# NVIDIA-AI-IOT/redtail

Hardware: AMD Instinct MI355X
Metric: stereo pairs/sec, ResNet18-2D 1257x369 (higher is better)
Workload: dtype f32

## Files before the change

### redtail_amd/csrc/kernels/conv_split.hip.h

```cpp
#pragma once
#include <type_traits>
#include "common.hip.h"
#include "conv_mfma.hip.h"

namespace rt {

constexpr float kSplitScale = 2048.f;
constexpr float kSplitInv = 1.f / 2048.f;

struct S3Split {
    f16x4 hi, lo;
};
__device__ static __forceinline__ S3Split s3_split(f32x4 v) {
    S3Split s;
#ifdef HIPEMU
#pragma unroll
    for (int j = 0; j < 4; j++) {
        const _Float16 h = (_Float16)v[j];
        s.hi[j] = h;
        s.lo[j] = (_Float16)((v[j] - (float)h) * kSplitScale);
    }
#else
    unsigned h[2], l[2];
#pragma unroll
// ... 182 lines not shown
                for (int e = 0; e < 4; e++)
                    o[e] = apply_act_fast(fmaf(acc_c[4 * q + e], kSplitInv, acc_m[4 * q + e]) + (bias4[q][e] + rr[q][e]), decltype(ACT)::value);
                if constexpr (YIL) {
                    const unsigned vo = (inb && 8 * q + 4 * kg < p.Cout) ? (unsigned)((oy * p.y_ystride + ox) * 4 + 4 * kg * cs32) * 4u : kBufOOB;
                    buf_store4(o, rs_y, vo, (unsigned)(8 * q * cs32) * 4u);
                } else {
                    const unsigned vo = inb ? (unsigned)(oy * p.y_ystride + ox * p.y_xstride + 4 * kg * cs32) * 4u : kBufOOB;
#pragma unroll
                    for (int e = 0; e < 4; e++)
                        buf_store(o[e], rs_y, (8 * q + 4 * kg + e < p.Cout) ? vo : kBufOOB, (unsigned)((8 * q + e) * cs32) * 4u);
                }
            }
        };
        if (act == 1) epilogue(std::integral_constant<int, 1>{});
        else if (act == 2) epilogue(std::integral_constant<int, 2>{});
        else epilogue(std::integral_constant<int, 0>{});
        RT_TSTAMP();
    }
#ifdef RT_KERNEL_TIMING
    __builtin_amdgcn_s_waitcnt(0);
    if (dbgp && tid == 0) { dbgp[14] = __builtin_amdgcn_s_memtime(); dbgp[15] = __builtin_amdgcn_s_memrealtime() - rt0; }
#endif
}

}

namespace rt {

template <int KH, int KW, int S, int NW_ = 4>
struct S3Cfg {
    static constexpr int NW = NW_, TY = NW_, TX = 32, CC = 16, TAPS = KH * KW, NT = 64 * NW_;
    static constexpr int PR = (TY - 1) * S + KH, PC = (TX - 1) * S + KW;
    static constexpr int PCH = (PC + 1) / 2;
    static constexpr int PCL = S == 2 ? 2 * PCH : PC;
    static constexpr int NPART = NW / 4;
    static constexpr int NPIX = PR * PC, NKP = ((NPIX + NPART - 1) / NPART + 63) / 64;
    static constexpr int PXB = 80;
    static constexpr int W_SLOTS = TAPS * 2 * 2 * 32;
    static constexpr int NK_W = (W_SLOTS + NT - 1) / NT;
    static constexpr int IN_BYTES = PR * PCL * PXB, GRP_BYTES = IN_BYTES + W_SLOTS * 16;
    static constexpr int KS_MAX = NW_ != 4 ? 1 : (S == 2 ? 2 : 4);
    static constexpr int max_groups(int want) {
        int ks = want < 1 ? 1 : (want > KS_MAX ? KS_MAX : want);
        while (ks > 1 && (ks == 3 || ks * GRP_BYTES < (ks - 1) * NW * 64 * 16 * 4)) ks--;
        return ks;
    }
    static_assert(IN_BYTES % 16 == 0, "weight image alignment");
    static_assert(S == 1 || S == 2, "stride 1 or 2");
};

#ifndef RT_S3_WAVES
#define RT_S3_WAVES(S) ((S) == 2 ? 2 : 4)
#endif
template <int KH, int KW, int S, bool XIL, bool YIL, int NW = 4, typename TIN = float, typename TOUT = float>
__global__ void __launch_bounds__(64 * NW * (S3Cfg<KH, KW, S, NW>::KS_MAX)) RT_WAVES_PER_EU(RT_S3_WAVES(S)) conv_s3_kernel(ConvArgs p) {
    using Cfg = S3Cfg<KH, KW, S, NW>;
    constexpr bool XF16 = std::is_same<TIN, _Float16>::value, YF16 = std::is_same<TOUT, _Float16>::value;
    constexpr unsigned ESX = Io<TIN>::ES, ESY = Io<TOUT>::ES;
    static_assert(!XIL || !XF16, "interleaved fp16 input: conv_f16mma_kernel");
    constexpr int TY = Cfg::TY, TX = Cfg::TX, CC = Cfg::CC, TAPS = Cfg::TAPS, PC = Cfg::PC, PCL = Cfg::PCL, PXB = Cfg::PXB;
    constexpr int NKP = Cfg::NKP, NK_W = Cfg::NK_W, NT = Cfg::NT;

    constexpr int IN_BYTES = Cfg::IN_BYTES, GRP_BYTES = Cfg::GRP_BYTES;
#ifdef HIPEMU
    HIP_DYNAMIC_SHARED(char, smem)
#else
    extern __shared__ __attribute__((aligned(16))) char smem[];
#endif

    const int tid_wg = threadIdx.x;
    const int KS = Cfg::KS_MAX == 1 ? 1 : __builtin_amdgcn_readfirstlane((int)blockDim.x / NT);
    const int kgi = Cfg::KS_MAX == 1 ? 0 : __builtin_amdgcn_readfirstlane(tid_wg / NT);
    const int tid = tid_wg - kgi * NT;
    char* const sIn = smem + kgi * GRP_BYTES;
    f32x4* const sW = reinterpret_cast<f32x4*>(smem + kgi * GRP_BYTES + IN_BYTES);
#ifdef RT_KERNEL_TIMING
    unsigned long long* dbgp = (p.dbg && kgi == 0) ? p.dbg + ((size_t)(blockIdx.z * gridDim.y + blockIdx.y) * gridDim.x + blockIdx.x) * 16 : nullptr;
    int dbi = 0;
    const unsigned long long rt0 = __builtin_amdgcn_s_memrealtime();
#endif
    RT_TSTAMP();
    const int lane = tid & 63;
    const int kg = lane >> 5, l31 = lane & 31;
    const int wv = __builtin_amdgcn_readfirstlane(tid >> 6);

    RT_WG_TILE_NB(p, tile, zi, n, nblk)
    const int tx0 = (tile % p.tiles_x) * TX;
    const int ty0 = (tile / p.tiles_x) * TY;
    const char* __restrict__ xb = elem_ptr(p.x, (int64_t)n * p.x_bstride, ESX);
    const int nchunks = p.CinPad / CC;
    int pad_y = p.pad_y, pad_x = p.pad_x, Ho = p.Ho, Wo = p.Wo, ch_row = zi;
    int64_t y_off = p.y_off + (int64_t)zi * p.y_zstride, w_off = 0, r_off = y_off, r_off_il8 = y_off;
    int64_t y_off_il4 = 4 * p.y_off + (int64_t)zi * p.y_zstride, r_off_il4 = y_off_il4;
    unsigned tap_mask = ~0u;
    if (p.zs) {
        const ZSlice z = p.zs[zi];
        pad_y = z.pad_y; pad_x = z.pad_x; Ho = z.Ho; Wo = z.Wo; ch_row = z.ch_row; y_off = z.y_off; w_off = z.w_off;
        r_off = z.r_off; r_off_il8 = z.r_off_il8;
        y_off_il4 = 4 * z.y_off;
        r_off_il4 = z.r_off_il4;
        tap_mask = z.tap_mask;
    }
    const int act = p.act;

    const int sg = wv & 3, spart = wv >> 2;
    const int* __restrict__ tab = p.ch_off + (int64_t)ch_row * p.CinPad + 4 * sg;
    unsigned voff[NKP];
    int lidx[NKP], xcol[NKP];
    const int* __restrict__ shtab = p.ch_shift ? p.ch_shift + (int64_t)ch_row * p.CinPad + 4 * sg : nullptr;
#pragma unroll
    for (int k = 0; k < NKP; k++) {
        const int pidx = spart * (NKP * 64) + lane + 64 * k;
        const int pr = pidx / PC, pc = pidx - pr * PC;
        const int iy = ty0 * S - pad_y + pr, ix = tx0 * S - pad_x + pc;
        const bool own = pidx < Cfg::NPIX && lane + 64 * k < NKP * 64;
        xcol[k] = ix;
        voff[k] = (own && iy >= 0 && iy < p.Hi && ix >= 0 && ix < p.Wi) ? (unsigned)(iy * p.x_pitch + ix) * (XIL ? 16u : ESX) : kBufOOB;
        const int col = S == 2 ? (pc & 1) * Cfg::PCH + (pc >> 1) : pc;
        lidx[k] = own ? (pr * PCL + col) * PXB + sg * 8 : -1;
    }
    const char* __restrict__ wsrc = reinterpret_cast<const char*>(p.w) + (w_off + ((int64_t)nblk * nchunks) * Cfg::W_SLOTS) * 16;
    const buf_rsrc rs_w = make_buf(wsrc);

    f32x4 rin[NKP];
    f32x4 rw[NK_W];
// ... 61 lines not shown
        const buf_rsrc rs_r = make_buf(elem_ptr(p.resid, r_il ? (int64_t)n * p.r_bstride + (YF16 ? r_off_il8 : r_off_il4) : rbase, ESY));
        if (r_il && YF16) {
            const unsigned vo = inb ? (unsigned)((oy * p.y_ystride + ox * p.y_xstride) * 8 + 4 * kg) * 2u : kBufOOB;
#pragma unroll
            for (int q = 0; q < 4; q++) {
                const u32x2_t u = __builtin_amdgcn_raw_buffer_load_b64(rs_r, (cb + 8 * q + 4 * kg < p.Cout) ? vo : kBufOOB, (unsigned)((cb + 8 * q) * rs32) * 2u, 0);
#pragma unroll
                for (int e = 0; e < 4; e++) rr[q][e] = (float)__builtin_bit_cast(_Float16, (unsigned short)(u[e >> 1] >> (16 * (e & 1))));
            }
        } else if (r_il) {
            const unsigned vo = inb ? (unsigned)((oy * p.y_ystride + ox * p.y_xstride) * 4 + 4 * kg * rs32) * 4u : kBufOOB;
#pragma unroll
            for (int q = 0; q < 4; q++) rr[q] = buf_load4(rs_r, (cb + 8 * q + 4 * kg < p.Cout) ? vo : kBufOOB, (unsigned)((cb + 8 * q) * rs32) * 4u);
        } else {
            const unsigned vo = inb ? (unsigned)(oy * p.y_ystride + ox * p.y_xstride + 4 * kg * rs32) * ESY : kBufOOB;
#pragma unroll
            for (int q = 0; q < 4; q++)
#pragma unroll
                for (int e = 0; e < 4; e++)
                    rr[q][e] = Io<TOUT>::load(rs_r, (cb + 8 * q + 4 * kg + e < p.Cout) ? vo : kBufOOB, (unsigned)((cb + 8 * q + e) * rs32) * ESY);
        }
    } else {
#pragma unroll
        for (int q = 0; q < 4; q++) rr[q] = f32x4{0.f, 0.f, 0.f, 0.f};
    }

    f32x16 acc_m, acc_c;
#pragma unroll
    for (int r = 0; r < 16; r++) { acc_m[r] = 0.f; acc_c[r] = 0.f; }
    const int a_off = kg * 32 + l31;
    const bool w_exact = p.w_exact != 0;
    const int b_off = (wv * S * PCL + l31) * PXB + kg * 16;
    auto compute = [&]() {
#pragma unroll
        for (int t = 0; t < TAPS; t++) {
            if (!((tap_mask >> t) & 1u)) continue;
            const int r = t / KW, s = t % KW;
            const int col = S == 2 ? (s & 1) * Cfg::PCH + (s >> 1) : s;
            const char* bp = sIn + b_off + (r * PCL + col) * PXB;
            const f16x8 bh = *reinterpret_cast<const f16x8*>(bp);
            const f16x8 ah = __builtin_bit_cast(f16x8, sW[a_off + (t * 2 + 0) * 64]);
            acc_m = __builtin_amdgcn_mfma_f32_32x32x16_f16(ah, bh, acc_m, 0, 0, 0);
            if (!w_exact) {
                const f16x8 al = __builtin_bit_cast(f16x8, sW[a_off + (t * 2 + 1) * 64]);
                acc_c = __builtin_amdgcn_mfma_f32_32x32x16_f16(al, bh, acc_c, 0, 0, 0);
            }
            if constexpr (!XF16) {
                const f16x8 bl = *reinterpret_cast<const f16x8*>(bp + 32);
                acc_c = __builtin_amdgcn_mfma_f32_32x32x16_f16(ah, bl, acc_c, 0, 0, 0);
            }
        }
    };

    if (kgi < nchunks) prefetch(kgi);
    RT_TSTAMP();
    for (int ch = kgi; ch < nchunks + kgi; ch += KS) {
        const bool mine = KS == 1 || ch < nchunks;
        if (ch != kgi) __syncthreads();
        if (mine) stage_to_lds();
        __syncthreads();
        RT_TSTAMP();
        if (ch + KS < nchunks) prefetch(ch + KS);
        if (mine) compute();
        RT_TSTAMP();
    }

#pragma unroll
    for (int r = 0; r < 16; r++) acc_m[r] = fmaf(acc_c[r], kSplitInv, acc_m[r]);
    if (KS > 1) {
        f32x4* const red = reinterpret_cast<f32x4*>(smem);
        __syncthreads();
        if (kgi > 0) {
#pragma unroll
            for (int q = 0; q < 4; q++)
                red[(((kgi - 1) * NW + wv) * 4 + q) * 64 + lane] = f32x4{acc_m[4 * q], acc_m[4 * q + 1], acc_m[4 * q + 2], acc_m[4 * q + 3]};
        }
        __syncthreads();
        if (kgi > 0) return;
        for (int g = 1; g < KS; g++)
#pragma unroll
            for (int q = 0; q < 4; q++) {
                const f32x4 v = red[(((g - 1) * NW + wv) * 4 + q) * 64 + lane];
#pragma unroll
                for (int e = 0; e < 4; e++) acc_m[4 * q + e] += v[e];
            }
    }

    const buf_rsrc rs_y = make_buf(elem_ptr(p.y, (YIL && !YF16) ? (int64_t)n * p.y_bstride + y_off_il4 : ybase, ESY));
    auto epilogue = [&](auto ACT) {
#pragma unroll
        for (int q = 0; q < 4; q++) {
            const f32x4 bv = *reinterpret_cast<const f32x4*>(p.bias + cb + 8 * q + 4 * kg);
            f32x4 o;
#pragma unroll
            for (int e = 0; e < 4; e++)
                o[e] = apply_act_fast(acc_m[4 * q + e] + (bv[e] + rr[q][e]), decltype(ACT)::value);
            if constexpr (YIL && YF16) {
                const unsigned vo = (inb && cb + 8 * q + 4 * kg < p.Cout) ? (unsigned)((oy * p.y_ystride + ox * p.y_xstride) * 8 + 4 * kg) * 2u : kBufOOB;
                u32x2_t w2;
#pragma unroll
                for (int e = 0; e < 2; e++)
                    w2[e] = (unsigned)__builtin_bit_cast(unsigned short, (_Float16)o[2 * e]) | ((unsigned)__builtin_bit_cast(unsigned short, (_Float16)o[2 * e + 1]) << 16);
                __builtin_amdgcn_raw_buffer_store_b64(w2, rs_y, vo, (unsigned)((cb + 8 * q) * cs32) * 2u, 0);
            } else if constexpr (YIL) {
                const unsigned vo = (inb && cb + 8 * q + 4 * kg < p.Cout) ? (unsigned)((oy * p.y_ystride + ox * p.y_xstride) * 4 + 4 * kg * cs32) * 4u : kBufOOB;
                buf_store4(o, rs_y, vo, (unsigned)((cb + 8 * q) * cs32) * 4u);
            } else {
                const unsigned vo = inb ? (unsigned)(oy * p.y_ystride + ox * p.y_xstride + 4 * kg * cs32) * ESY : kBufOOB;
#pragma unroll
                for (int e = 0; e < 4; e++)
                    Io<TOUT>::store(o[e], rs_y, (cb + 8 * q + 4 * kg + e < p.Cout) ? vo : kBufOOB, (unsigned)((cb + 8 * q + e) * cs32) * ESY);
            }
        }
    };
    if (act == 1) epilogue(std::integral_constant<int, 1>{});
    else if (act == 2) epilogue(std::integral_constant<int, 2>{});
    else epilogue(std::integral_constant<int, 0>{});
    RT_TSTAMP();
// ... 392 lines not shown
```

### redtail_amd/csrc/rt_capi.hip

```cpp
#include <hip/hip_runtime.h>

#include <algorithm>
#include <atomic>
#include <cmath>
#include <cstdarg>
#include <cstdio>
#include <cstdlib>
#include <cstring>
#include <string>
#include <map>
#include <mutex>
#include <vector>

#include "../../include/rt_stereo.h"
#if defined(__HIP_DEVICE_COMPILE__) && !defined(RT_BUILT_NO_SLP)
#error "rt_capi.hip must be compiled with -fno-slp-vectorize -DRT_BUILT_NO_SLP (redtail_amd/build.py: DEVICE_FLAGS)"
#endif
#include "kernels/common.hip.h"
#include "kernels/conv_mfma.hip.h"
#include "kernels/conv_wino.hip.h"
#include "kernels/deconv3d_small.hip.h"
#include "kernels/imgproc.hip.h"
#include "kernels/rectify.hip.h"
#include "kernels/decode.hip.h"
// ... 1063 lines not shown
namespace {


struct SubConv {
    int KH = 1, KW = 1, S = 1, NBW = 1, CC = 8;
    int TY = 4, TXW = 2, NW = 4, WLDS = 1;
    int CinPad = 0, Cout = 0;
    int Hi = 0, Wi = 0, Ho = 0, Wo = 0, pad_y = 0, pad_x = 0, nz = 1;
    int x_pitch = 0;
    std::vector<rt::ZSlice> zs_host;
    int64_t y_cstride = 0, y_zstride = 0, y_off = 0;
    int64_t r_cstride = 0;
    int y_ystride = 0, y_xstride = 1;
    float* w_dev = nullptr;
    int* choff_dev = nullptr;
    int w_exact = 0;
    int* shift_dev = nullptr;
    rt::ZSlice* zs_dev = nullptr;
    int direct = 0, cin_real = 0;
    int wino = 0;
    int x_f16 = 0, y_f16 = 0;
    int f16mma = 0;
    int x_il8 = 0, y_il8 = 0, r_il8 = 0;
    int dp4 = 0;
    int f16first = 0;
    int split3 = 0;
    int rb = 0;
    int s3first = 0;
    int s3p = 0;
    int small3d = 0;
    rt::Deconv3dSmallArgs s3{};
    std::vector<float> small_w;
    void* small_il_dev = nullptr;
    int small_il_f32 = 0;
};

}

struct FoldFactor {
    rtConvPlan* pl = nullptr;
    rtConvPlan* pr = nullptr;
    float* wedge_dev = nullptr;
    int F = 0, K = 0, D = 0, H = 0, W = 0;
    int64_t a_elems = 0, c_elems = 0, t_elems = 0, e_elems = 0;
    std::mutex mu;
    std::map<rtStream, std::pair<void*, size_t>> own;
};

struct ConvKnobs {
    int xcd = 1, trace = 0;
    int rb_tiles = 0;
    int rbs_seg = 0;
    int ksplit = -1;
    int s3p_grid = 0;
    int zinner = 1;
    int nbinner = 1;
    int dw = -1;
    int dw_nseg = 0;
    int fold_u = 2;
    int f16p_walk = -1;
    int f16p_classes = 1;
    int small_walk = -1;
    int r4 = -1;
};

struct rtConvPlan {
    std::vector<SubConv> subs;
    FoldFactor* ff = nullptr;
    mutable std::once_flag env_once;
    mutable ConvKnobs opt;
    int softarg = 0;
    float* bias_dev = nullptr;
    float* zeros_dev = nullptr;
    int act = 0, has_resid = 0, dtype = RT_F32;
    int out_dims[4] = {0, 0, 0, 1};
    int64_t x_bstride = 0, y_bstride = 0;
    int64_t r_bstride = 0;
    int is2d = 0, cin = 0, hin = 0, win = 0;
    std::vector<float> w_canon;
    rtConv2dDesc desc2d{};
    int is_deconv = 0;
    int in_pitch = 0, out_pitch = 0;
    float* rb_w1_dev = nullptr;
    float* rb_bias1_dev = nullptr;
    int rb_act1 = 0, rb_cmid = 0;
    float* rbd_w1_dev = nullptr;
    float* rbd_w2_dev = nullptr;
    int x_split = 0, y_split = 0;
    float* rbh_w1_dev = nullptr;
    float* rbh_w2_dev = nullptr;
    int w_f16 = 0;
    int is_conv3d = 0, is_deconv3d = 0;
    int c3d_C = 0, c3d_cin = 0, c3d_dchw = 0, c3d_fold = 0;
    int c3d_dw = 0;
    rtConv3dDesc desc3d{};
    int in_dims3[3] = {0, 0, 0};
    int flags = 0;
};

namespace {

struct Phase1D {
    int K = 0;
    int pad = 0;
    int tap[8] = {0};
};
// ... 117 lines not shown
                    const int nb = co / 32, cc = co % 32, ch = ci / 16, h = (ci % 16) / 8, e = ci % 8;
                    packed[(size_t)base * 8 + ((((((size_t)nb * nch + ch) * taps + (u * sc.KW + v)) * 2 + h) * 32 + cc) * 8) + e] = bits;
                }
    return base;
}

int upload_zslices(SubConv& sc, const std::vector<rt::ZSlice>& zs) {
    RT_HIP(hipMalloc((void**)&sc.zs_dev, zs.size() * sizeof(rt::ZSlice)));
    RT_HIP(hipMemcpy(sc.zs_dev, zs.data(), zs.size() * sizeof(rt::ZSlice), hipMemcpyHostToDevice));
    return 0;
}

int upload_table(SubConv& sc, const std::vector<int>& table) {
    RT_HIP(hipMalloc((void**)&sc.choff_dev, table.size() * sizeof(int)));
    RT_HIP(hipMemcpy(sc.choff_dev, table.data(), table.size() * sizeof(int), hipMemcpyHostToDevice));
    return 0;
}

int upload_bias(rtConvPlan* plan, const float* bias, int n) {
    const int padded = rt::round_up(n, 64);
    std::vector<float> b(padded + 64, 0.f);
    if (bias) std::memcpy(b.data(), bias, n * sizeof(float));
    RT_HIP(hipMalloc((void**)&plan->bias_dev, b.size() * sizeof(float)));
    RT_HIP(hipMemcpy(plan->bias_dev, b.data(), b.size() * sizeof(float), hipMemcpyHostToDevice));
    plan->zeros_dev = plan->bias_dev + padded;
    return 0;
}

bool window_supported(int KH, int KW, int S) {
    if (S == 1) return (KH == 3 && KW == 3) || (KH <= 2 && KW <= 2 && KH >= 1 && KW >= 1);
    if (S == 2) return (KH == 3 && KW == 3) || (KH == 5 && KW == 5);
    return false;
}

bool dev_knobs() {
    static const bool on = [] { const char* e = getenv("RT_DEV_KNOBS"); return e && atoi(e) != 0; }();
    return on;
}
int env_int(const char* name, int dflt) {
    if (!dev_knobs()) return dflt;
    const char* e = getenv(name);
    return e ? atoi(e) : dflt;
}

#ifdef RT_EXPERIMENTAL
inline int exp_knob(const char* name, int dflt) { return env_int(name, dflt); }
#else
inline int exp_knob(const char*, int dflt) { return dflt; }
#endif
ConvKnobs read_conv_knobs() {
    ConvKnobs k;
    k.xcd = env_int("RT_CONV_XCD", k.xcd); k.trace = env_int("RT_CONV_TRACE", k.trace);
    k.rb_tiles = exp_knob("RT_RB_TILES", k.rb_tiles); k.rbs_seg = env_int("RT_RBS_SEG", k.rbs_seg); k.ksplit = env_int("RT_S3_KSPLIT", k.ksplit);
    k.s3p_grid = env_int("RT_S3P_GRID", k.s3p_grid); k.zinner = env_int("RT_Z_INNER", k.zinner); k.nbinner = env_int("RT_NB_INNER", k.nbinner);
    k.dw = env_int("RT_F16_DW", k.dw); k.dw_nseg = env_int("RT_DW_NSEG", k.dw_nseg); k.fold_u = env_int("RT_FOLD_U", k.fold_u);
    k.f16p_walk = env_int("RT_F16P_WALK", k.f16p_walk); k.f16p_classes = env_int("RT_F16P_CLASSES", k.f16p_classes);
    k.small_walk = env_int("RT_SMALL_IL_WALK", k.small_walk); k.r4 = env_int("RT_F16_R4", k.r4);
    return k;
}
thread_local int tl_exact_fp32 = 0;
int exact_fp32() { return tl_exact_fp32 || env_int("RT_CONV_EXACT_FP32", 0) != 0; }
struct ExactScope {
    int prev;
    explicit ExactScope(int flags) : prev(tl_exact_fp32) { tl_exact_fp32 = (flags & RT_CONV_EXACT_FP32) ? 1 : prev; }
    ~ExactScope() { tl_exact_fp32 = prev; }
};

void set_tile(SubConv& sc, int variant) {
    switch (variant) {
        case 0: sc.TY = 4; sc.TXW = 2; sc.NW = 4; break;
        case 4: sc.TY = 2; sc.TXW = 2; sc.NW = 4; break;
        case 9: sc.TY = 2; sc.TXW = 1; sc.NW = 2; break;
        case 8: sc.TY = 8; sc.TXW = 1; sc.NW = 8; break;
        case 10: sc.TY = 8; sc.TXW = 1; sc.NW = 4; break;
        default: sc.TY = 4; sc.TXW = 1; sc.NW = 4; break;
    }
    sc.WLDS = 1;
}

int64_t count_wgs(const SubConv& sc) {
    return rt::cdiv(sc.Ho, sc.TY) * rt::cdiv(sc.Wo, 32 * sc.TXW) * rt::cdiv(sc.Cout, 32 * sc.NBW) * sc.nz;
}

void check_direct(SubConv& sc, int cin_real) {
    const bool win = (sc.KH == sc.KW && (sc.KH == 1 || sc.KH == 2 || sc.KH == 3 || sc.KH == 5)) ||
                     (sc.KH == 1 && sc.KW == 2) || (sc.KH == 2 && sc.KW == 1);
    if (!win || (int64_t)sc.Cout * cin_real * sc.KH * sc.KW > 4096) sc.direct = 0;
}

void choose_tiling(SubConv& sc, bool allow_wino = true) {
    sc.direct = (sc.Cout <= 2 && env_int("RT_CONV_NO_DIRECT", 0) == 0) ? 1 : 0;
    sc.CC = 8;
    sc.NBW = 1;
    if (sc.KH == 5) sc.CC = 4;
    const int forced = env_int("RT_CONV_VARIANT", -1);
    set_tile(sc, forced >= 0 ? forced : 6);
    sc.wino = (allow_wino && !sc.direct && sc.KH == 3 && sc.KW == 3 && sc.S == 1 && sc.Cout >= 24 && env_int("RT_CONV_NO_WINO", 0) == 0) ? 1 : 0;
    if (sc.wino) { sc.CC = 8; sc.NBW = 1; sc.TY = exp_knob("RT_WINO_WAVES", 4); sc.TXW = 1; sc.NW = sc.TY; }
    const int nbw = env_int("RT_CONV_NBW", 0);
    if (nbw == 1 || (nbw == 2 && sc.KH != 5)) sc.NBW = nbw;
    const bool s3_win = (sc.KH == 3 && sc.KW == 3 && (sc.S == 1 || sc.S == 2)) || (sc.S == 1 && sc.KH <= 2 && sc.KW <= 2);
    sc.split3 = (!sc.direct && s3_win && !exact_fp32() && env_int("RT_NO_S3", 0) == 0) ? 1 : 0;
    if (sc.split3) {
        sc.wino = 0; sc.CC = 16; sc.NBW = 1; sc.TY = 4; sc.TXW = 1; sc.NW = 4;
        if (sc.KH == 3 && sc.KW == 3 && sc.S == 1 && exp_knob("RT_S3_ROWS", 4) == 8) sc.TY = sc.NW = 8;
    }
// ... 17 lines not shown
                packed[(((((size_t)t * 2 + c) * 2 + 1) * 2 + kg) * 32 + co) * 8 + e] = lo;
            }
    if (int rc = upload_weights(sc, packed)) return rc;
    sc.s3p = 1; sc.split3 = 0; sc.wino = 0;
    sc.CinPad = 32; sc.CC = 16; sc.NBW = 1; sc.TXW = 1; sc.TY = sc.NW = 8;
    return 0;
}

bool s3first_eligible(const SubConv& sc, int cin, int has_resid) {
    return !sc.direct && sc.KH == 5 && sc.KW == 5 && sc.S == 2 && cin <= 3 && !has_resid && sc.nz == 1 &&
           !exact_fp32() && env_int("RT_NO_S3", 0) == 0;
}
template <typename F>
int upload_s3first(SubConv& sc, int cin_real, F wfun) {
    const int nblk = (int)rt::cdiv(sc.Cout, 32);
    std::vector<uint16_t> packed((size_t)nblk * rt::S3FirstCfg::W_SLOTS * 8, 0);
    for (int co = 0; co < sc.Cout; co++)
        for (int c = 0; c < cin_real; c++)
            for (int r = 0; r < 5; r++)
                for (int sx = 0; sx < 5; sx++) {
                    uint16_t hi, lo;
                    split_f16(wfun(co, c, r, sx), hi, lo);
                    const int k = 3 * sx + c, h = k / 8, e = k % 8;
                    const size_t blk = (size_t)(co / 32) * rt::S3FirstCfg::W_SLOTS * 8;
                    packed[blk + ((((size_t)r * 2 + 0) * 2 + h) * 32 + co % 32) * 8 + e] = hi;
                    packed[blk + ((((size_t)r * 2 + 1) * 2 + h) * 32 + co % 32) * 8 + e] = lo;
                }
    if (int rc = upload_weights(sc, packed)) return rc;
    sc.s3first = 1; sc.s3p = 0; sc.split3 = 0; sc.wino = 0;
    sc.NBW = 1; sc.TXW = 1; sc.TY = sc.NW = 4;
    return 0;
}

template <bool Z, int PAT>
bool drop_structural_zeros(std::vector<float>& packed) {
    using Taps = rt::SmallTaps<Z, PAT>;
    constexpr int NJ = Taps::NJ;
    if (env_int("RT_NO_SMALL_SPARSE", 0) != 0) return false;
    const size_t rows = packed.size() / (NJ * NJ);
    for (size_t r = 0; r < rows; r++)
        for (int f = 0; f < NJ; f++)
            for (int j = 0; j < NJ; j++)
                if (!Taps::valid(f, j) && packed[(r * NJ + f) * NJ + j] != 0.f) return false;
    std::vector<float> dense(rows * Taps::NV);
    for (size_t r = 0; r < rows; r++)
        for (int f = 0; f < NJ; f++)
            for (int j = 0; j < NJ; j++)
                if (Taps::valid(f, j)) dense[r * Taps::NV + Taps::index(f, j)] = packed[(r * NJ + f) * NJ + j];
    packed.swap(dense);
    return true;
}

template <typename T> constexpr const char* type_tag() { return sizeof(T) == 2 ? "f16" : "f32"; }
template <int KH, int KW, int S, bool XIL, bool YIL, int NW = 4, typename TIN = float, typename TOUT = float>
void launch_s3(dim3 grid, int ks, int64_t per_cu, hipStream_t st, const rt::ConvArgs& a, int trace = 0) {
    using Cfg = rt::S3Cfg<KH, KW, S, NW>;
    ks = Cfg::max_groups(ks);
    while (ks > 1 && std::min<int64_t>(per_cu, 4) * ks * Cfg::GRP_BYTES > 160 * 1024) ks = Cfg::max_groups(ks - 1);
    if (trace)
        fprintf(stderr, "[rt] conv_s3<%d,%d,%d,%d,%d,%d,%s,%s> r%d grid %u x %u x %u ks %d\n", KH, KW, S, (int)XIL, (int)YIL, NW, type_tag<TIN>(),
                type_tag<TOUT>(), a.r_il8, grid.x, grid.y, grid.z, ks);
#ifndef HIPEMU
    static std::atomic<unsigned long long> done{0};
    int dev = 0;
    if (hipGetDevice(&dev) == hipSuccess && dev >= 0 && dev < 64 && !((done.load(std::memory_order_acquire) >> dev) & 1ull)) {
        (void)hipFuncSetAttribute(reinterpret_cast<const void*>(&rt::conv_s3_kernel<KH, KW, S, XIL, YIL, NW, TIN, TOUT>),
                                  hipFuncAttributeMaxDynamicSharedMemorySize, Cfg::KS_MAX * Cfg::GRP_BYTES);
        done.fetch_or(1ull << dev, std::memory_order_release);
    }
#endif
    hipLaunchKernelGGL((rt::conv_s3_kernel<KH, KW, S, XIL, YIL, NW, TIN, TOUT>), grid, dim3(64 * NW * ks), (size_t)ks * Cfg::GRP_BYTES, st, a);
}

int device_cus() {
    static std::atomic<int> cus[64];
    int dev = 0;
    if (hipGetDevice(&dev) != hipSuccess || dev < 0 || dev >= 64) return 256;
    int n = cus[dev].load(std::memory_order_relaxed);
    if (!n) {
        hipDeviceProp_t prop;
        n = (hipGetDeviceProperties(&prop, dev) == hipSuccess && prop.multiProcessorCount > 0) ? prop.multiProcessorCount : 256;
        cus[dev].store(n, std::memory_order_relaxed);
    }
    return n;
}

std::vector<float> to_f32(const void* w, size_t n, int dtype) {
    std::vector<float> out(n);
    if (dtype == RT_F16) {
        const char* h = static_cast<const char*>(w);
        for (size_t i = 0; i < n; i++) {
            _Float16 v;
            std::memcpy(&v, h + 2 * i, 2);
            out[i] = (float)v;
        }
    } else {
        std::memcpy(out.data(), w, n * sizeof(float));
    }
    return out;
}

template <int KH, int KW, int S, int NBW, int CC>
int launch_window(const SubConv& sc, const rt::ConvArgs& a, dim3 grid, hipStream_t st) {
#define RT_TILE(ty, txw, nw, wlds)                                                                        \
    if (sc.TY == ty && sc.TXW == txw && sc.NW == nw && sc.WLDS == (wlds ? 1 : 0)) {                       \
        hipLaunchKernelGGL((rt::conv_mfma_f32_kernel<KH, KW, S, ty, txw, NBW, CC, nw, wlds>), grid,       \
                           dim3(64 * nw), 0, st, a);                                                      \
        return 0;                                                                                         \
    }
    if (sc.y_il8) return 1;
    if (sc.x_f16 || sc.y_f16) {
        if (!(sc.TY == 4 && sc.TXW == 1 && sc.NW == 4 && sc.WLDS) || !sc.y_f16) return 1;
        if (sc.x_f16)
            hipLaunchKernelGGL((rt::conv_mfma_f32_kernel<KH, KW, S, 4, 1, NBW, CC, 4, true, _Float16, _Float16>), grid, dim3(256), 0, st, a);
        else
            hipLaunchKernelGGL((rt::conv_mfma_f32_kernel<KH, KW, S, 4, 1, NBW, CC, 4, true, float, _Float16>), grid, dim3(256), 0, st, a);
        return 0;
    }
    RT_TILE(4, 2, 4, true) RT_TILE(4, 1, 4, true) RT_TILE(2, 2, 4, true) RT_TILE(2, 1, 2, true) RT_TILE(8, 1, 8, true) RT_TILE(8, 1, 4, true)
#undef RT_TILE
    return 1;
}

int launch_sub(const SubConv& sc, const rt::ConvArgs& a, dim3 grid, hipStream_t st) {
// ... 1615 lines not shown
}

int enqueue_s3first(const Launch& L, const SubConv& sc, const rt::ConvArgs& a, const ConvGrid& g) {
    if (L.plan->opt.trace) fprintf(stderr, "[rt] conv_s3_first<%d> grid %u x %u x %u twin %d\n", sc.y_il8 ? 1 : 0, g.grid.x, g.grid.y, g.grid.z, a.x2 ? 1 : 0);
    if (sc.y_il8) hipLaunchKernelGGL((rt::conv_s3_first_kernel<true>), g.grid, dim3(256), 0, S(L.s), a);
    else hipLaunchKernelGGL((rt::conv_s3_first_kernel<false>), g.grid, dim3(256), 0, S(L.s), a);
    RT_LAUNCH_CHECK("conv_s3_first_kernel");
    return 0;
}

int enqueue_f16first(const Launch& L, const SubConv& sc, const rt::ConvArgs& a, const ConvGrid& g) {
    if (L.plan->opt.trace) fprintf(stderr, "[rt] conv_f16_first<%d> grid %u x %u x %u twin %d\n", sc.y_il8 ? 1 : 0, g.grid.x, g.grid.y, g.grid.z, a.x2 ? 1 : 0);
    if (sc.y_il8) hipLaunchKernelGGL((rt::conv_f16_first_kernel<true>), g.grid, dim3(256), 0, S(L.s), a, L.plan->cin);
    else hipLaunchKernelGGL((rt::conv_f16_first_kernel<false>), g.grid, dim3(256), 0, S(L.s), a, L.plan->cin);
    RT_LAUNCH_CHECK("conv_f16_first_kernel");
    return 0;
}

int enqueue_split3(const Launch& L, const SubConv& sc, const rt::ConvArgs& a, const ConvGrid& g) {
    const rtConvPlan* plan = L.plan;
    const dim3 grid = g.fold(g.grid);
    const int trace = plan->opt.trace;
    bool launched = false;
    int ks = 1;
    const int64_t per_cu = rt::cdiv((int64_t)g.grid.x * g.grid.y * (g.gz / L.batch), (int64_t)device_cus());
    if (plan->opt.ksplit > 0 || (plan->opt.ksplit < 0 && !(L.hints & RT_HINT_THROUGHPUT))) {
        const int nch = a.CinPad / 16;
        ks = plan->opt.ksplit > 0 ? plan->opt.ksplit : (per_cu == 1 && nch >= 4 ? 4 : (per_cu <= 2 && nch >= 2 ? 2 : 1));
    }
    if (sc.x_f16 || sc.y_f16) {
        if (!sc.x_f16 && sc.x_il8 && sc.KH == 3 && sc.KW == 3 && sc.S == 1 && sc.TY == 4 && sc.y_f16) {
            if (sc.y_il8) launch_s3<3, 3, 1, true, true, 4, float, _Float16>(grid, ks, per_cu, S(L.s), a, trace);
            else launch_s3<3, 3, 1, true, false, 4, float, _Float16>(grid, ks, per_cu, S(L.s), a, trace);
            RT_LAUNCH_CHECK("conv_s3_kernel<float, f16>");
            return 0;
        }
        RT_REQUIRE(!sc.x_il8 && !(sc.y_il8 && sc.x_f16) && sc.TY == 4 && sc.y_f16, "rt_conv_enqueue: fp16-storage variant of the split kernel not instantiated");
#define RT_S3H(kh, kw, st)                                                                                           \
    if (!launched && sc.KH == kh && sc.KW == kw && sc.S == st) {                                                     \
        if (sc.x_f16) launch_s3<kh, kw, st, false, false, 4, _Float16, _Float16>(grid, ks, per_cu, S(L.s), a, trace); \
        else if (sc.y_il8) launch_s3<kh, kw, st, false, true, 4, float, _Float16>(grid, ks, per_cu, S(L.s), a, trace); \
        else launch_s3<kh, kw, st, false, false, 4, float, _Float16>(grid, ks, per_cu, S(L.s), a, trace);            \
        launched = true;                                                                                             \
    }
        RT_S3H(3, 3, 1) RT_S3H(3, 3, 2) RT_S3H(1, 1, 1) RT_S3H(1, 2, 1) RT_S3H(2, 1, 1) RT_S3H(2, 2, 1)
#undef RT_S3H
    }
#ifdef RT_EXPERIMENTAL
    if (!launched && sc.KH == 3 && sc.KW == 3 && sc.S == 1 && sc.TY == 8) {
        with_bools([&](auto xi, auto yi) { launch_s3<3, 3, 1, xi, yi, 8>(grid, ks, per_cu, S(L.s), a, trace); }, sc.x_il8, sc.y_il8);
        launched = true;
    }
#endif
#define RT_S3(kh, kw, st)                                                                                                              \
    if (!launched && sc.KH == kh && sc.KW == kw && sc.S == st) {                                                                       \
        with_bools([&](auto xi, auto yi) { launch_s3<kh, kw, st, xi, yi>(grid, ks, per_cu, S(L.s), a, trace); }, sc.x_il8, sc.y_il8); \
        launched = true;                                                                                                               \
    }
    RT_S3(3, 3, 1) RT_S3(3, 3, 2) RT_S3(1, 1, 1) RT_S3(1, 2, 1) RT_S3(2, 1, 1) RT_S3(2, 2, 1)
#undef RT_S3
    if (!launched) return fail(RT_E_UNSUPPORTED, "conv (split fp16): window %dx%d stride %d not instantiated", sc.KH, sc.KW, sc.S);
    RT_LAUNCH_CHECK("conv_s3_kernel");
    return 0;
}

int enqueue_f16dw(const Launch& L, const SubConv& sc, rt::ConvArgs& a, bool& taken) {
    const rtConvPlan* plan = L.plan;
    if (!(plan->c3d_dw && plan->opt.dw != 0 && sc.KH == 3 && sc.KW == 3 && sc.S == 1 && sc.x_il8 && sc.y_il8 && !sc.zs_dev && sc.y_xstride == 1 &&
          (!plan->has_resid || sc.r_il8) && (plan->act == RT_ACT_NONE || plan->act == RT_ACT_ELU) && !sc.shift_dev))
        return 0;
    using Dw = rt::ConvF16DwCfg;
    const int dw_tiles_x = (int)rt::cdiv(sc.Wo, Dw::TX), dw_nkb = (int)rt::cdiv(sc.Cout, 32);
    const int64_t npairs = rt::cdiv(dw_tiles_x * (int)rt::cdiv(sc.Ho, Dw::TY), 2);
    int nseg = plan->opt.dw_nseg;
    double best = 1e30, fill = 1.0;
    for (int ns = 1; ns <= sc.nz; ns++) {
        const int seg = (int)rt::cdiv(sc.nz, ns);
        if (ns > 1 && seg < 4) break;
        if ((int)rt::cdiv(sc.nz, seg) != ns || (plan->opt.dw_nseg > 0 && ns != std::min(plan->opt.dw_nseg, sc.nz))) continue;
        const int64_t wgs = npairs * ns * dw_nkb * L.batch, rounds = rt::cdiv(wgs, (int64_t)device_cus());
        const double steps = seg + (ns > 1 ? 3.0 : 1.7), cost = (double)rounds * steps;
        if (cost < best - 1e-9) { best = cost; nseg = ns; fill = (double)wgs / (double)(rounds * device_cus()) * seg / steps; }
    }
    if (plan->opt.dw < 0 && fill < 0.6) return 0;
    taken = true;
    nseg = std::max(1, std::min(nseg, sc.nz));
    a.tiles_x = dw_tiles_x;
    a.dw_ntiles = a.tiles_x * (int)rt::cdiv(sc.Ho, Dw::TY);
    a.dw_cpc = plan->c3d_C / 16;
    a.nb_inner = dw_nkb;
    a.dw_seg = (int)rt::cdiv(sc.nz, nseg);
    a.dw_nseg = (int)rt::cdiv(sc.nz, a.dw_seg);
    const int64_t gx = npairs * a.dw_nseg * a.nb_inner;
    RT_REQUIRE(gx < (1ll << 31) && L.batch <= 65535, "rt_conv_enqueue: grid limit exceeded");
    dim3 gd((unsigned)gx, 1u, (unsigned)L.batch);
    const bool resident = a.dw_cpc <= 2, elu = plan->act == RT_ACT_ELU;
    if (plan->opt.trace)
        fprintf(stderr, "[rt] conv_f16dw<%d,%d,%d> grid %u x %u segments %d x %d slices, %d chunks per slice\n", resident ? 1 : 0,
                plan->has_resid ? 1 : 0, elu ? 1 : 0, gd.x, gd.z, a.dw_nseg, a.dw_seg, a.dw_cpc);
    with_bools([&](auto res, auto hr, auto el) { hipLaunchKernelGGL((rt::conv_f16dw_kernel<res, hr, el>), gd, dim3(512), 0, S(L.s), a); },
               resident, plan->has_resid, elu);
    RT_LAUNCH_CHECK("conv_f16dw_kernel");
    return 0;
}

int enqueue_f16mma(const Launch& L, const SubConv& sc, rt::ConvArgs& a, const ConvGrid& g) {
    const rtConvPlan* plan = L.plan;
    bool taken = false;
    if (int rc = enqueue_f16dw(L, sc, a, taken)) return rc;
    if (taken) return 0;
    if (sc.KH == 3 && sc.KW == 3 && sc.S == 1 && sc.x_il8 && sc.y_il8 && !sc.zs_dev && sc.TY == 4 && sc.y_xstride == 1 &&
        (plan->opt.r4 > 0 || (plan->opt.r4 < 0 && plan->is_conv3d && sc.Ho >= 12))) {
// ... 363 lines not shown
```

Baseline: 2821.

## Add deep-pipelined split-fp16 conv variant with double register prefetch and tap lookahead

Adds a DEEP template form of the split-fp16 conv kernel that keeps two channel chunks in flight in registers (ping-pong buffers) and prefetches each tap's LDS operands one tap ahead of its MFMAs. The host picks it automatically for interleaved fp32 inputs when the grid gives only one or two workgroups per CU and there are enough chunks. The aim is to hide global-load and LDS latency in low-occupancy launches where k-splitting is not used. It costs extra VGPRs (a second prefetch buffer plus the lookahead operands) and adds more kernel instantiations.

```diff
diff --git a/redtail_amd/csrc/kernels/conv_split.hip.h b/redtail_amd/csrc/kernels/conv_split.hip.h
--- a/redtail_amd/csrc/kernels/conv_split.hip.h
+++ b/redtail_amd/csrc/kernels/conv_split.hip.h
@@ -258,9 +258,10 @@
 #ifndef RT_S3_WAVES
 #define RT_S3_WAVES(S) ((S) == 2 ? 2 : 4)
 #endif
-template <int KH, int KW, int S, bool XIL, bool YIL, int NW = 4, typename TIN = float, typename TOUT = float>
-__global__ void __launch_bounds__(64 * NW * (S3Cfg<KH, KW, S, NW>::KS_MAX)) RT_WAVES_PER_EU(RT_S3_WAVES(S)) conv_s3_kernel(ConvArgs p) {
+template <int KH, int KW, int S, bool XIL, bool YIL, int NW = 4, typename TIN = float, typename TOUT = float, bool DEEP = false>
+__global__ void __launch_bounds__(64 * NW * (DEEP ? 1 : S3Cfg<KH, KW, S, NW>::KS_MAX)) RT_WAVES_PER_EU(DEEP ? 2 : RT_S3_WAVES(S)) conv_s3_kernel(ConvArgs p) {
     using Cfg = S3Cfg<KH, KW, S, NW>;
+    static_assert(!DEEP || (XIL && std::is_same<TIN, float>::value && std::is_same<TOUT, float>::value), "the deep form: interleaved fp32 input, fp32 output");
     constexpr bool XF16 = std::is_same<TIN, _Float16>::value, YF16 = std::is_same<TOUT, _Float16>::value;
     constexpr unsigned ESX = Io<TIN>::ES, ESY = Io<TOUT>::ES;
     static_assert(!XIL || !XF16, "interleaved fp16 input: conv_f16mma_kernel");
@@ -275,8 +276,8 @@
 #endif
 
     const int tid_wg = threadIdx.x;
-    const int KS = Cfg::KS_MAX == 1 ? 1 : __builtin_amdgcn_readfirstlane((int)blockDim.x / NT);
-    const int kgi = Cfg::KS_MAX == 1 ? 0 : __builtin_amdgcn_readfirstlane(tid_wg / NT);
+    const int KS = (Cfg::KS_MAX == 1 || DEEP) ? 1 : __builtin_amdgcn_readfirstlane((int)blockDim.x / NT);
+    const int kgi = (Cfg::KS_MAX == 1 || DEEP) ? 0 : __builtin_amdgcn_readfirstlane(tid_wg / NT);
     const int tid = tid_wg - kgi * NT;
     char* const sIn = smem + kgi * GRP_BYTES;
     f32x4* const sW = reinterpret_cast<f32x4*>(smem + kgi * GRP_BYTES + IN_BYTES);
@@ -444,6 +445,90 @@
         }
     };
 
+    if constexpr (DEEP) {
+        struct Ops { f16x8 bh, bl, ah, al; };
+        auto fetch = [&](int t) {
+            const int r = t / KW, s = t % KW;
+            const int col = S == 2 ? (s & 1) * Cfg::PCH + (s >> 1) : s;
+            const char* bp = sIn + b_off + (r * PCL + col) * PXB;
+            Ops o;
+            o.bh = *reinterpret_cast<const f16x8*>(bp);
+            o.bl = *reinterpret_cast<const f16x8*>(bp + 32);
+            o.ah = __builtin_bit_cast(f16x8, sW[a_off + (t * 2 + 0) * 64]);
+            o.al = __builtin_bit_cast(f16x8, sW[a_off + (t * 2 + 1) * 64]);
+            return o;
+        };
+        auto compute_ahead = [&]() {
+            Ops nx = fetch(0);
+#pragma unroll
+            for (int t = 0; t < TAPS; t++) {
+                const Ops o = nx;
+                if (t + 1 < TAPS) nx = fetch(t + 1);
+                __builtin_amdgcn_sched_barrier(0);
+                if ((tap_mask >> t) & 1u) {
+                    acc_m = __builtin_amdgcn_mfma_f32_32x32x16_f16(o.ah, o.bh, acc_m, 0, 0, 0);
+                    if (!w_exact) acc_c = __builtin_amdgcn_mfma_f32_32x32x16_f16(o.al, o.bh, acc_c, 0, 0, 0);
+                    acc_c = __builtin_amdgcn_mfma_f32_32x32x16_f16(o.ah, o.bl, acc_c, 0, 0, 0);
+                }
+                __builtin_amdgcn_sched_barrier(0);
+            }
+        };
+        f32x4 rin1[NKP];
+        f32x4 rw1[NK_W];
+        auto prefetch_to = [&](int ch, f32x4 (&ri)[NKP], f32x4 (&rv)[NK_W]) {
+            const int off = tab[ch * CC];
+            const buf_rsrc rs = make_buf(xb, off >= 0);
+#pragma unroll
+            for (int k = 0; k < NKP; k++) ri[k] = buf_load4(rs, voff[k], (unsigned)off * 4u);
+            const unsigned so = (unsigned)ch * (unsigned)(Cfg::W_SLOTS * 16);
+#pragma unroll
+            for (int k = 0; k < NK_W; k++) {
+                const int idx = tid + NT * k;
+                rv[k] = buf_load4(rs_w, idx < Cfg::W_SLOTS ? (unsigned)idx * 16u : kBufOOB, so);
+            }
+        };
+        auto stage_from = [&](const f32x4 (&ri)[NKP], const f32x4 (&rv)[NK_W]) {
+#pragma unroll
+            for (int k = 0; k < NKP; k++) {
+                if (lidx[k] < 0) continue;
+                const S3Split sp = s3_split(ri[k]);
+                *reinterpret_cast<f16x4*>(sIn + lidx[k]) = sp.hi;
+                *reinterpret_cast<f16x4*>(sIn + lidx[k] + 32) = sp.lo;
+            }
+#pragma unroll
+            for (int k = 0; k < NK_W; k++) {
+                const int idx = tid + NT * k;
+                if (idx < Cfg::W_SLOTS) sW[idx] = rv[k];
+            }
+        };
+        auto round = [&](int ch, int next, f32x4 (&ri)[NKP], f32x4 (&rv)[NK_W]) {
+            if (ch != 0) __syncthreads();
+            stage_from(ri, rv);
+            __syncthreads();
+            RT_TSTAMP();
+            if (next >= 0) prefetch_to(next, ri, rv);
+            compute_ahead();
+            RT_TSTAMP();
+        };
+        if (nchunks < 2) {
+            prefetch_to(0, rin, rw);
+            RT_TSTAMP();
+            round(0, -1, rin, rw);
+        } else {
+            prefetch_to(0, rin, rw);
+            prefetch_to(1, rin1, rw1);
+            RT_TSTAMP();
+            int ch = 0;
+            for (; ch + 3 < nchunks; ch += 2) {
+                round(ch, ch + 2, rin, rw);
+                round(ch + 1, ch + 3, rin1, rw1);
+            }
+            const bool three = nchunks - ch == 3;
+            round(ch, three ? ch + 2 : -1, rin, rw);
+            round(ch + 1, -1, rin1, rw1);
+            if (three) round(ch + 2, -1, rin, rw);
+        }
+    } else {
     if (kgi < nchunks) prefetch(kgi);
     RT_TSTAMP();
     for (int ch = kgi; ch < nchunks + kgi; ch += KS) {
@@ -456,6 +541,7 @@
         if (mine) compute();
         RT_TSTAMP();
     }
+    }
 
 #pragma unroll
     for (int r = 0; r < 16; r++) acc_m[r] = fmaf(acc_c[r], kSplitInv, acc_m[r]);
diff --git a/redtail_amd/csrc/rt_capi.hip b/redtail_amd/csrc/rt_capi.hip
--- a/redtail_amd/csrc/rt_capi.hip
+++ b/redtail_amd/csrc/rt_capi.hip
@@ -1139,6 +1139,7 @@
     int rb_tiles = 0;
     int rbs_seg = 0;
     int ksplit = -1;
+    int s3_deep = -1;
     int s3p_grid = 0;
     int zinner = 1;
     int nbinner = 1;
@@ -1362,6 +1363,7 @@
     ConvKnobs k;
     k.xcd = env_int("RT_CONV_XCD", k.xcd); k.trace = env_int("RT_CONV_TRACE", k.trace);
     k.rb_tiles = exp_knob("RT_RB_TILES", k.rb_tiles); k.rbs_seg = env_int("RT_RBS_SEG", k.rbs_seg); k.ksplit = env_int("RT_S3_KSPLIT", k.ksplit);
+    k.s3_deep = env_int("RT_S3_DEEP", k.s3_deep);
     k.s3p_grid = env_int("RT_S3P_GRID", k.s3p_grid); k.zinner = env_int("RT_Z_INNER", k.zinner); k.nbinner = env_int("RT_NB_INNER", k.nbinner);
     k.dw = env_int("RT_F16_DW", k.dw); k.dw_nseg = env_int("RT_DW_NSEG", k.dw_nseg); k.fold_u = env_int("RT_FOLD_U", k.fold_u);
     k.f16p_walk = env_int("RT_F16P_WALK", k.f16p_walk); k.f16p_classes = env_int("RT_F16P_CLASSES", k.f16p_classes);
@@ -1485,24 +1487,26 @@
 }
 
 template <typename T> constexpr const char* type_tag() { return sizeof(T) == 2 ? "f16" : "f32"; }
-template <int KH, int KW, int S, bool XIL, bool YIL, int NW = 4, typename TIN = float, typename TOUT = float>
+template <int KH, int KW, int S, bool XIL, bool YIL, int NW = 4, typename TIN = float, typename TOUT = float, bool DEEP = false>
 void launch_s3(dim3 grid, int ks, int64_t per_cu, hipStream_t st, const rt::ConvArgs& a, int trace = 0) {
     using Cfg = rt::S3Cfg<KH, KW, S, NW>;
-    ks = Cfg::max_groups(ks);
+    constexpr int KS_MAX = DEEP ? 1 : Cfg::KS_MAX;
+    ks = DEEP ? 1 : Cfg::max_groups(ks);
     while (ks > 1 && std::min<int64_t>(per_cu, 4) * ks * Cfg::GRP_BYTES > 160 * 1024) ks = Cfg::max_groups(ks - 1);
     if (trace)
         fprintf(stderr, "[rt] conv_s3<%d,%d,%d,%d,%d,%d,%s,%s> r%d grid %u x %u x %u ks %d\n", KH, KW, S, (int)XIL, (int)YIL, NW, type_tag<TIN>(),
                 type_tag<TOUT>(), a.r_il8, grid.x, grid.y, grid.z, ks);
+    if (trace > 1) fprintf(stderr, "[rt] conv_s3 form: %s\n", DEEP ? "deep" : "plain");
 #ifndef HIPEMU
     static std::atomic<unsigned long long> done{0};
     int dev = 0;
     if (hipGetDevice(&dev) == hipSuccess && dev >= 0 && dev < 64 && !((done.load(std::memory_order_acquire) >> dev) & 1ull)) {
-        (void)hipFuncSetAttribute(reinterpret_cast<const void*>(&rt::conv_s3_kernel<KH, KW, S, XIL, YIL, NW, TIN, TOUT>),
-                                  hipFuncAttributeMaxDynamicSharedMemorySize, Cfg::KS_MAX * Cfg::GRP_BYTES);
+        (void)hipFuncSetAttribute(reinterpret_cast<const void*>(&rt::conv_s3_kernel<KH, KW, S, XIL, YIL, NW, TIN, TOUT, DEEP>),
+                                  hipFuncAttributeMaxDynamicSharedMemorySize, KS_MAX * Cfg::GRP_BYTES);
         done.fetch_or(1ull << dev, std::memory_order_release);
     }
 #endif
-    hipLaunchKernelGGL((rt::conv_s3_kernel<KH, KW, S, XIL, YIL, NW, TIN, TOUT>), grid, dim3(64 * NW * ks), (size_t)ks * Cfg::GRP_BYTES, st, a);
+    hipLaunchKernelGGL((rt::conv_s3_kernel<KH, KW, S, XIL, YIL, NW, TIN, TOUT, DEEP>), grid, dim3(64 * NW * ks), (size_t)ks * Cfg::GRP_BYTES, st, a);
 }
 
 int device_cus() {
@@ -3224,12 +3228,20 @@
         launched = true;
     }
 #endif
-#define RT_S3(kh, kw, st)                                                                                                              \
+    const int nch_s3 = a.CinPad / 16;
+    const bool deep = ks == 1 && sc.x_il8 && sc.TY == 4 && !a.ch_shift &&
+                      (plan->opt.s3_deep > 0 || (plan->opt.s3_deep < 0 && ((per_cu == 1 && nch_s3 >= 2) || (per_cu == 2 && nch_s3 >= 8))));
+#define RT_S3(kh, kw, st, has_deep)                                                                                                    \
     if (!launched && sc.KH == kh && sc.KW == kw && sc.S == st) {                                                                       \
-        with_bools([&](auto xi, auto yi) { launch_s3<kh, kw, st, xi, yi>(grid, ks, per_cu, S(L.s), a, trace); }, sc.x_il8, sc.y_il8); \
+        with_bools([&](auto xi, auto yi) {                                                                                             \
+            if constexpr (has_deep && decltype(xi)::value) {                                                                           \
+                if (deep) return launch_s3<kh, kw, st, true, yi, 4, float, float, true>(grid, 1, per_cu, S(L.s), a, trace);           \
+            }                                                                                                                          \
+            launch_s3<kh, kw, st, xi, yi>(grid, ks, per_cu, S(L.s), a, trace);                                                         \
+        }, sc.x_il8, sc.y_il8);                                                                                                        \
         launched = true;                                                                                                               \
     }
-    RT_S3(3, 3, 1) RT_S3(3, 3, 2) RT_S3(1, 1, 1) RT_S3(1, 2, 1) RT_S3(2, 1, 1) RT_S3(2, 2, 1)
+    RT_S3(3, 3, 1, true) RT_S3(3, 3, 2, true) RT_S3(1, 1, 1, false) RT_S3(1, 2, 1, false) RT_S3(2, 1, 1, false) RT_S3(2, 2, 1, true)
 #undef RT_S3
     if (!launched) return fail(RT_E_UNSUPPORTED, "conv (split fp16): window %dx%d stride %d not instantiated", sc.KH, sc.KW, sc.S);
     RT_LAUNCH_CHECK("conv_s3_kernel");
```

After: 2818. Within noise of the previous version (-0.1%).
